# yangao07/LAMSA

Hardware: AMD Instinct MI355X
Metric: aligned Gbase/s, 10 kbp ONT-error reads (12%: sub/ins/del 4% each), -T ont2d vs GRCh37-sized stand-in; inputs resident in HBM when the timed region starts (upload excluded: see pcie_inclusive_*) (higher is better)
Workload: dtype int32

## Files before the change

### lamsa_amd/csrc/hp_align_api.hip

```cpp
#include <hip/hip_runtime.h>
#include <algorithm>
#include <atomic>
#include <map>
#include <mutex>
#include <stdlib.h>
#include <string.h>
#include <time.h>
#include "hp_phase.h"
#include "hp_handle.h"
#include "hp_hostprep.h"

using namespace hp;

#ifndef HP_WAVES_PER_SIMD
#define HP_WAVES_PER_SIMD 4
#endif
__global__ __launch_bounds__(64, HP_WAVES_PER_SIMD) void k_align_batch(AlignArgs a)
{
    __shared__ int32_t lds[HP_BOTH_LDS_WORDS];
    const int slot = blockIdx.x;
    for (;;) {
        int u = 0;
        if (wv::leader()) u = atomicAdd(a.counter, 1);
        u = wv::uni(u);
// ... 411 lines not shown
    S->valid = true;
    return LAMSA_HP_OK;
}

static int cap_waves(int n_waves, size_t slab_per_wave, int n_cu)
{
    static const size_t budget = []() { size_t f = 0, t = 0; if (hipMemGetInfo(&f, &t) != hipSuccess || t == 0) { t = (size_t)288 << 30; f = t; } return std::min(t / 4, f / 3); }();
    if (slab_per_wave * (size_t)n_waves <= budget) return n_waves;
    size_t fit = budget / (slab_per_wave ? slab_per_wave : 1);
    if (n_cu > 0 && fit >= (size_t)n_cu) fit -= fit % (size_t)n_cu;
    return fit < 1 ? 1 : (int)fit;
}

#ifdef HP_PROF
static void prof_report(Slot &T, const long long *d_prof, int n)
{
    if (!d_prof) return;
    {
        std::vector<long long> pr((size_t)n * 64);
        hipMemcpy(pr.data(), d_prof, sizeof(long long) * pr.size(), hipMemcpyDeviceToHost);
        if (const char *dump = getenv("LAMSA_HP_PROF_DUMP")) {
            if (FILE *fp = fopen(dump, "wb")) {
                for (int r = 0; r < n; ++r) { long long hl[2] = {T.h_H[r], T.h_len[r]}; fwrite(hl, 8, 2, fp); fwrite(&pr[(size_t)r * 64], 8, 64, fp); }
                fclose(fp);
            }
        }
        std::vector<int> idx((size_t)n); for (int i = 0; i < n; ++i) idx[i] = i;
        auto tot = [&](int r) { long long t = 0; for (int k = 0; k < 6; ++k) t += pr[(size_t)r * 64 + k]; return t; };
        std::sort(idx.begin(), idx.end(), [&](int x, int y) { return tot(x) > tot(y); });
        long long sum[64] = {0}; for (int r = 0; r < n; ++r) for (int k = 0; k < 64; ++k) sum[k] += pr[(size_t)r * 64 + k];
        fprintf(stderr, "[HP_PROF] cycles: setup chain1 fill1 chain2 fill2 publish | in chain1: init+minext mainscan track pop-loop bound+flines | o_l H\n");
        fprintf(stderr, "[HP_PROF] SUM  "); for (int k = 0; k < 11; ++k) fprintf(stderr, " %lld", sum[k] / 1000000); fprintf(stderr, " (Mcycles) targets %lld trips %lld init_Mcyc %lld\n", sum[11], sum[12], sum[13] / 1000000);
#ifdef HP_PROF_TRACK
        fprintf(stderr, "[HP_PROF] branch tracking (-DHP_PROF_TRACK: the line_build stamps below are off): marking pass %lld Mcyc; %lld seeds visited; %lld tracks, %lld Mcyc in them, %lld steps up; "
                        "%lld arrivals at a node with several sons, %lld Mcyc in cut_branch\n", sum[16] / 1000000, sum[19], sum[18], sum[17] / 1000000, sum[20], sum[21], sum[22] / 1000000);
#endif
        fprintf(stderr, "[HP_PROF] line_build: %lld lines (%lld without a gap), %lld anchors, %lld gaps | Mcyc: anchor walk %lld, gap list %lld, gaps in lanes %lld, gaps one by one %lld, assembly %lld\n",
                sum[21], sum[22], sum[12], sum[23], sum[16] / 1000000, sum[17] / 1000000, sum[18] / 1000000, sum[19] / 1000000, sum[20] / 1000000);
        fprintf(stderr, "[HP_PROF] gaps: %lld in lines with fewer than HP_GAP_MIN gaps (%lld lines with gaps); lane gaps: %lld hits scanned, %lld refused (range too long or too many active hits)\n", sum[54], sum[55], sum[11], sum[13]);
        { const char *nm[] = {"ksw_global", "ksw_extend", "backtrack", "ref_fetch", "head_fix", "frag_extend", "split_mapping", "tail_fix", "res_split", "res_aux", "mini_line_regs", "sort index"};
          for (int k = 0; k < 12; ++k) fprintf(stderr, "[HP_PROF] %-16s %8lld Mcyc %10lld calls\n", nm[k], sum[24 + 2 * k] / 1000000, sum[25 + 2 * k]);
#ifdef HP_PROF_FILL
          fprintf(stderr, "[HP_PROF] in frags_merge: boundary repair (merge_cigar_full) %lld Mcyc %lld calls; junctions through split_mapping %lld Mcyc %lld calls; fragments of several seeds %lld Mcyc %lld calls; 64-step gathers %lld Mcyc %lld\n", sum[16] / 1000000, sum[17], sum[18] / 1000000, sum[19], sum[20] / 1000000, sum[21], sum[22] / 1000000, sum[23]);
#endif
          fprintf(stderr, "[HP_PROF] direction-matrix bytes in HBM %lld (%lld jobs); hits passed through nodes_per_init %lld (%lld calls)\n", sum[52], sum[53], sum[54], sum[55]);
          fprintf(stderr, "[HP_PROF] chain_first start: seed loop %lld, node_set loop %lld, min_extend %lld Mcyc (%lld reads with a MIN pass)\n", sum[56] / 1000000, sum[57] / 1000000, sum[58] / 1000000, sum[59]);
          fprintf(stderr, "[HP_PROF] query <= 62: ksw_extend %lld Mcyc %lld calls, ksw_global %lld Mcyc %lld calls\n", sum[60] / 1000000, sum[61], sum[62] / 1000000, sum[63]);
          const char *bn[] = {"[bi_extend total]", "[bi_extend after left ext]", "17-32", "33-64", "65-128", "129-256", "257-512", ">512"};
          for (int k = 0; k < 2; ++k) fprintf(stderr, "[HP_PROF] ksw_extend qlen %-8s %8lld Mcyc %10lld calls\n", bn[k], sum[48 + 2 * k] / 1000000, sum[49 + 2 * k]); }
        {
            std::vector<long long> pd((size_t)n * 64);
            hipMemcpy(pd.data(), d_prof + ((size_t)n + 1) * 64, sizeof(long long) * pd.size(), hipMemcpyDeviceToHost);
            long long sd[64] = {0}; for (int r = 0; r < n; ++r) for (int k = 0; k < 64; ++k) sd[k] += pd[(size_t)r * 64 + k];
            const char *cn[] = {"one set, q <= 62", "packed, one set", "packed, two sets", "band 1 set slides", "band 2 sets slides", "band 4 sets slides", "int32 sets", "LDS / HBM rows",
                                "band 1 set fixed", "band 2 sets fixed", "band 4 sets fixed"};
            for (int c = 0; c < 11; ++c) fprintf(stderr, "[HP_PROF] wave jobs, ksw_extend %-18s %8lld Mcyc %10lld Mcells %9lld calls %10lld rows\n", cn[c], sd[4 * c] / 1000000, sd[4 * c + 1] / 1000000, sd[4 * c + 2], sd[4 * c + 3]);
            fprintf(stderr, "[HP_PROF] wave jobs, junctions of the class 'band 2 sets fixed': %lld jobs, wj_run %lld Mcyc of which staging %lld; ksw_bi_extend %lld Mcyc of which after the left extension %lld; "
                            "in ksw_extend_band<2>: setup and first fill %lld, rows %lld, backtrack %lld Mcyc\n",
                    sd[51], sd[50] / 1000000, sd[49] / 1000000, sd[47] / 1000000, sd[48] / 1000000, sd[44] / 1000000, sd[45] / 1000000, sd[46] / 1000000);
        }
        for (int q = 0; q < 8 && q < n; ++q) { int r = idx[q]; fprintf(stderr, "[HP_PROF] read %d L=%d:", r, T.h_len[r]); for (int k = 0; k < 11; ++k) fprintf(stderr, " %lld", pr[(size_t)r * 64 + k] / 1000000); fprintf(stderr, " | o_l %lld H %lld | targets %lld trips %lld init_Mcyc %lld\n", pr[(size_t)r * 64 + 14], pr[(size_t)r * 64 + 15], pr[(size_t)r * 64 + 11], pr[(size_t)r * 64 + 12], pr[(size_t)r * 64 + 13] / 1000000); }
    }
}
#endif

struct PhasedLayout { size_t bytes, o[15]; int unit_cap, lj_cap, wj_cap; int64_t fl_cap, line_cap, job_cap; };
static PhasedLayout phased_layout(int n, int64_t n_hits, int64_t n_bases, int64_t stream_cap)
// ... 193 lines not shown
    const int n = T.n_reads;
    for (float &v : h->kernel_ms) v = 0;
    S->r_st.assign((size_t)n + 1, 0); S->r_off.assign((size_t)n + 1, 0); S->r_len.assign((size_t)n + 1, 0); S->r_tb.assign((size_t)n + 1, 0); S->r_work.assign(4 * (size_t)n + 4, 0);
    if (S->stream.ensure(64)) { h->err = "hipHostMalloc(results)"; return LAMSA_HP_ENOMEM; }
    if (n == 0) {
        if (R) { R->stream = (const int32_t *)S->stream.p; R->stream_words = 0; R->read_off = S->r_off.data(); R->read_len = S->r_len.data(); R->read_status = S->r_st.data(); R->read_tbases = S->r_tb.data(); R->read_work = S->r_work.data(); }
        return LAMSA_HP_OK;
    }
    const double t_0 = now_s();
    HIPCHK(h, hipEventSynchronize(Ln.e1), LAMSA_HP_EKERNEL);
    const double t_1 = now_s();
    hipEventElapsedTime(&h->kernel_ms[0], Ln.e0, Ln.e1);
    if (Ln.phased) {
        hipEvent_t ev[6] = {Ln.e0, Ln.ep[0], Ln.ep[1], Ln.ep[2], Ln.ep[3], Ln.e1};
        for (int k = 0; k < 5; ++k) hipEventElapsedTime(&h->kernel_ms[2 + k], ev[k], ev[k + 1]);
        const unsigned long long *dg = Ln.out1.h_diag(n);
        for (int k = 0; k < 4; ++k) h->kernel_ms[7 + k] = dg[2 * k + 1] >= dg[2 * k] && dg[2 * k + 1] ? (float)((double)(dg[2 * k + 1] - dg[2 * k]) * 1e-5) : 0.f;
        h->kernel_ms[11] = (float)dg[8]; h->kernel_ms[12] = (float)dg[9];
        hipEventElapsedTime(&h->kernel_ms[13], Ln.ep[0], Ln.ep[4]);
        hipEventElapsedTime(&h->kernel_ms[14], Ln.ep[0], Ln.ep[5]);
        hipEventElapsedTime(&h->kernel_ms[15], Ln.ep[5], Ln.ep[6]);
        h->kernel_ms[16] = (float)dg[12]; h->kernel_ms[17] = (float)((double)dg[13] * 1e-6); h->kernel_ms[18] = (float)dg[14]; h->kernel_ms[19] = (float)((double)dg[15] * 4e-6); h->kernel_ms[20] = (float)((double)dg[16] * 1e-6);
#ifdef HP_PROF
        prof_report(T, (const long long *)Ln.prof.p, n);
#endif
    }
    memcpy(S->r_off.data(), Ln.out1.h_off(), 8 * (size_t)n); memcpy(S->r_len.data(), Ln.out1.h_len(n), 4 * (size_t)n);
    memcpy(S->r_st.data(), Ln.out1.h_st(n), 4 * (size_t)n); memcpy(S->r_tb.data(), Ln.out1.h_tb(n), 4 * (size_t)n); memcpy(S->r_work.data(), Ln.out1.h_work(n), 16 * (size_t)n);
    unsigned long long used1 = 0;
    for (int r = 0; r < n; ++r) if (S->r_off[r] >= 0 && (unsigned long long)(S->r_off[r] + S->r_len[r]) > used1) used1 = (unsigned long long)(S->r_off[r] + S->r_len[r]);
    if ((int64_t)used1 > Ln.out1.stream_cap) used1 = (unsigned long long)Ln.out1.stream_cap;
    std::vector<int32_t> again;
    for (int r = 0; r < n; ++r) if ((S->r_st[r] & LAMSA_HP_ST_OVERFLOW) || S->r_off[r] < 0) again.push_back(r);
    unsigned long long used2 = 0;
    if (!again.empty()) {
        int mL = 0, mH = 0; int64_t cap2 = 1024;
        for (int r : again) { mL = std::max(mL, T.h_len[r]); mH = std::max(mH, T.h_H[r]); cap2 += read_out_cap(T.h_len[r], 8, h->result_tags); }
        if (grow(h, S->out2.buf, 4 * (size_t)cap2 + 256) || S->out2.host.ensure(OutDev::hdr(n) + 256) || grow(h, S->retry_list, 4 * again.size())) { h->err = "hipMalloc(retry)"; return LAMSA_HP_ENOMEM; }
        S->out2.stream_cap = cap2;
        HIPCHK(h, hipMemcpyAsync(S->retry_list.p, again.data(), 4 * again.size(), hipMemcpyHostToDevice, Ln.cs), LAMSA_HP_EKERNEL);
        int rc = launch_align(h, S, T, Ln, S->out2, (const int32_t *)S->retry_list.p, (int)again.size(), 8, mL, mH, h->ev0, h->ev1, true);
        if (rc) return rc;
        hipEventElapsedTime(&h->kernel_ms[1], h->ev0, h->ev1);
        const int64_t *off2 = S->out2.h_off(); const int32_t *len2 = S->out2.h_len(n), *st2 = S->out2.h_st(n), *tb2 = S->out2.h_tb(n), *wk2 = S->out2.h_work(n);
        for (int r : again) if (off2[r] >= 0 && (unsigned long long)(off2[r] + len2[r]) > used2) used2 = (unsigned long long)(off2[r] + len2[r]);
        if ((int64_t)used2 > cap2) used2 = (unsigned long long)cap2;
        for (int r : again) { S->r_st[r] = st2[r]; S->r_len[r] = len2[r]; S->r_tb[r] = tb2[r]; for (int q = 0; q < 4; ++q) S->r_work[4 * r + q] = wk2[4 * r + q]; S->r_off[r] = off2[r] < 0 ? -1 : (int64_t)used1 + off2[r]; }
    }
    for (int r = 0; r < n; ++r) if (S->r_off[r] < 0) { S->r_off[r] = 0; S->r_len[r] = 0; S->r_st[r] |= LAMSA_HP_ST_OVERFLOW; }
    if (!R) return LAMSA_HP_OK;
    if (S->stream.ensure(4 * (size_t)(used1 + used2) + 64)) { h->err = "hipHostMalloc(results)"; return LAMSA_HP_ENOMEM; }
    int32_t *hs = (int32_t *)S->stream.p;
    if (used1) DL(hs, Ln.out1.stream(n), 4 * (size_t)used1);
    if (used2) DL(hs + used1, S->out2.stream(n), 4 * (size_t)used2);
    DLSYNC();
    if (g_trace) fprintf(stderr, "[lamsa_hp] collect: waited %.1f ms for the kernel (%.1f ms), results %.1f ms (%.2f GB)\n", 1e3 * (t_1 - t_0), h->kernel_ms[0], 1e3 * (now_s() - t_1), 4e-9 * (double)(used1 + used2));
    R->stream = hs; R->stream_words = (int64_t)(used1 + used2); R->read_off = S->r_off.data(); R->read_len = S->r_len.data(); R->read_status = S->r_st.data(); R->read_tbases = S->r_tb.data(); R->read_work = S->r_work.data();
    return LAMSA_HP_OK;
}
#undef DL
#undef DLSYNC

static int check_batch_args(lamsa_hp_handle *h, const lamsa_hp_batch *B)
{
    if (!h || !B || B->n_reads < 0) return LAMSA_HP_EINVAL;
    if (!h->d_pac) { h->err = "handle was created without a reference"; return LAMSA_HP_EINVAL; }
// ... 136 lines not shown
```

### lamsa_amd/csrc/hp_chain.h

```cpp
#pragma once
#include "hp_batch.h"
#include "hp_sort.h"

namespace hp {

enum { F_MATCH = 0, F_SPLIT_MATCH = 1, F_MISMATCH = 2, F_MATCH_THD = 2, F_LONG_MISMATCH = 3, F_INSERT = 4, F_DELETE = 5,
       F_CHR_DIF = 6, F_REVERSE = 7, F_UNCONNECT = 8, F_UNMATCH = 9, F_INIT = 20 };
enum { MIN_FLAG = 1, MULTI_FLAG = 2, UNLIMITED_FLAG = 3, WHOLE_FLAG = 4, TRACKED_FLAG = 5 };
enum { L_MERGB = 0, L_NMERG = 1, L_MERGH = 2, L_INTER = 4, L_DUMP = 8 };

HP_INL int score_table(int flag) { return flag <= 3 ? 1 : (flag <= 7 ? -3 : -6); }

#define HP_MAX_SLOTS 16383
#define HP_MAX_HITS_PER_SEED 16383

struct NodeS {
    int64_t pos;
    int32_t chr;
    int32_t slot_j;
    int16_t sid;
    int8_t strand, len_dif8;
    int8_t dp_flag;
    uint8_t son_flag;
    uint8_t match_flag;
// ... 509 lines not shown
{
    for (;;) {
        int l = 2 * i + 1, rr = 2 * (i + 1), m = i;
        if (l < ns.node_n && ns.node[l] < ns.node[i]) m = l;
        if (rr < ns.node_n && ns.node[rr] < ns.node[m]) m = rr;
        if (m == i) return;
        ns_swap(ns, i, m); i = m;
    }
}
HP_FN int ns_extract_minpos(NScore &ns)
{
    if (ns.node_n < 1) return -1;
    int m = ns.node[0];
    --ns.node_n;
    ns.node[0] = ns.node[ns.node_n]; ns.score[0] = ns.score[ns.node_n]; ns.NM[0] = ns.NM[ns.node_n];
    ns_minpos_sift(ns, 0);
    return m;
}
HP_FN int ns_add_bounded(NScore &ns, int node, int score, int NM)
{
    if (ns.node_n < ns.max_n) {
        ns.score[ns.node_n] = score; ns.NM[ns.node_n] = NM; ns.node[ns.node_n++] = node;
        if (ns.node_n == ns.max_n) for (int i = (ns.node_n - 1) / 2; i >= 0; --i) ns_min_sift(ns, i);
        return -1;
    }
    if (ns.score[0] < score || (ns.score[0] == score && ns.NM[0] > NM)) {
        int ret = ns.node[0];
        ns.score[0] = score; ns.NM[0] = NM; ns.node[0] = node;
        ns_min_sift(ns, 0);
        return ret;
    }
    return -2;
}
HP_FN void ns_add_end(ReadCtx &r, NScore &ns, int score, int NM, int node, const wv::Lane<int> *path = nullptr, int n_path = 0)
{
    if (score < ns.min_score_thd) return;
    if (ns.node_n >= ns.cap) { r.cx.status |= ST_OVERFLOW; return; }
    ns.score[ns.node_n] = score; ns.NM[ns.node_n] = NM; ns.node[ns.node_n++] = node;
    r.nd[node].dp_flag = TRACKED_FLAG;
    if (path) { HP_G NodeS *gd = (HP_G NodeS *)r.nd; WAVE_FOR(l) { if (l < n_path) gd[(*path)[l]].dp_flag = TRACKED_FLAG; } return; }
    for (int t = r.n_from[node]; t >= 0; t = r.n_from[t]) r.nd[t].dp_flag = TRACKED_FLAG;
}

HP_FN int best_son(ReadCtx &r, int f)
{
    int max_score = 0, max_NM = 0, max_dis = 0, flag_thd = F_INIT, max = -1;
    const int x = r.n_seed[f];
    for (int s = r.n_first[f], c = 0; c < r.n_son_n[f] && s >= 0; s = r.n_next[s], ++c) {
        const int mf = r.nd[s].match_flag, sx = r.n_seed[s];
        if (mf <= flag_thd && (r.n_max_score[s] > max_score || (r.n_max_score[s] == max_score && (sx - x < max_dis || r.n_max_NM[s] < max_NM)))) {
            max = s; max_score = r.n_max_score[s]; max_NM = r.n_max_NM[s]; max_dis = sx - x;
            if (mf <= F_MATCH_THD) flag_thd = F_MATCH_THD;
        }
    }
    return max;
}
HP_FN void detach(ReadCtx &r, int s, int max_node, NScore &ns)
{
    r.n_from[s] = -1;
    r.n_max_score[s] -= (r.nd[s].score - 1);
    r.n_max_NM[s] -= (r.nd[s].NM - r.h_nm[s]);
    r.n_node_n[max_node] -= (r.n_node_n[s] - 1);
    ns_add_end(r, ns, r.n_max_score[s], r.n_max_NM[s], max_node);
}
HP_INL void leaf_mark(ReadCtx &r, int f)
{
    if (r.leaf_on) { const int x = r.n_seed[f]; r.leaf_bits[x >> 5] |= (int)(1u << (x & 31)); }
}
HP_FN void cut_branch(ReadCtx &r, int f, NScore &ns)
{
    const int keep = best_son(r, f);
    if (keep < 0) { r.cx.status |= ST_REFEXIT; r.n_in_de[f] = 0; leaf_mark(r, f); return; }
    for (int s = r.n_first[f], c = 0, nn = r.n_son_n[f]; c < nn && s >= 0; ++c) {
        const int nxt = r.n_next[s];
        if (s != keep) detach(r, s, r.n_max_node[s], ns);
        s = nxt;
    }
    if (r.nd[f].score > r.n_max_score[keep]) {
        r.n_in_de[keep] = -1;
        detach(r, keep, r.n_max_node[keep], ns);
        r.n_son_n[f] = 0; r.n_first[f] = r.n_last[f] = -1;
        r.n_max_node[f] = f; r.n_max_score[f] = r.nd[f].score; r.n_max_NM[f] = r.nd[f].NM;
    } else {
        r.n_son_n[f] = 1; r.n_first[f] = r.n_last[f] = keep; r.n_next[keep] = -1;
        r.n_max_node[f] = r.n_max_node[keep]; r.n_max_score[f] = r.n_max_score[keep]; r.n_max_NM[f] = r.n_max_NM[keep];
    }
    r.n_in_de[f] = 0;
    leaf_mark(r, f);
}
HP_HOT void branch_track(ReadCtx &r, int n, NScore &ns)
{
    const HP_G int32_t *g_from = (const HP_G int32_t *)r.n_from, *g_son_n = (const HP_G int32_t *)r.n_son_n;
    const HP_G NodeS *g_nd = (const HP_G NodeS *)r.nd;
    HP_G int32_t *g_ms = (HP_G int32_t *)r.n_max_score, *g_mn = (HP_G int32_t *)r.n_max_NM, *g_mx = (HP_G int32_t *)r.n_max_node, *g_in_de = (HP_G int32_t *)r.n_in_de;
    int max_score, max_NM, max_node;
    g_in_de[n] = -1;
    const int n_sons = g_son_n[n], n_score = g_nd[n].score, n_NM = g_nd[n].NM;
    int fa = g_from[n];
    if (n_sons == 0) { max_node = n; max_score = n_score; max_NM = n_NM; }
    else { max_node = g_mx[n]; max_score = g_ms[n]; max_NM = g_mn[n]; }
    wv::Lane<int> path;
    WAVE_FOR(l) { path[l] = 0; }
    int n_path = 0; bool path_ok = n_sons == 0;
    int prev = n;
    while (fa >= 0) {
        const int fa_sons = g_son_n[fa], fa_score = g_nd[fa].score, fa_from = g_from[fa];
#ifdef HP_PROF_TRACK
        if (HP_PROF_CHAIN_ON && r.prof) r.prof[20] += 1;
#endif
        if (fa_sons == 1) {
            if (fa_score > max_score) {
                const int s = r.n_first[fa];
                g_ms[prev] = max_score; g_mn[prev] = max_NM; g_mx[prev] = max_node;
                wv::sync();
                r.n_in_de[s] = -1;
                detach(r, s, max_node, ns);
                r.n_son_n[fa] = 0; r.n_first[fa] = r.n_last[fa] = -1;
                max_score = r.nd[fa].score; max_NM = r.nd[fa].NM; max_node = fa;
                n_path = 0; path_ok = true;
            } else if (path_ok) {
                if (n_path < 64) { WAVE_FOR(l) { if (l == n_path) path[l] = fa; } ++n_path; } else path_ok = false;
            }
            prev = fa;
            fa = fa_from;
        } else {
            g_ms[prev] = max_score; g_mn[prev] = max_NM; g_mx[prev] = max_node;
            const int left_ = g_in_de[fa] - 1;
            g_in_de[fa] = left_;
#ifdef HP_PROF_TRACK
            if (HP_PROF_CHAIN_ON && r.prof) r.prof[21] += 1;
            const long long tcb_ = wv::clock();
#endif
            if (left_ == 0) { wv::sync(); cut_branch(r, fa, ns); }
#ifdef HP_PROF_TRACK
            if (HP_PROF_CHAIN_ON && r.prof) r.prof[22] += wv::clock() - tcb_;
#endif
            return;
        }
    }
    ns_add_end(r, ns, max_score, max_NM, max_node, path_ok ? &path : nullptr, n_path);
}

struct RunR { int lo, hi; };
HP_NOINL RunR reach_run(ReadCtx &r, int node, long long Rcap)
{
    const HP_G NodeS *ns = (const HP_G NodeS *)r.nd;
    const HP_G int32_t *g_srt = (const HP_G int32_t *)r.srt;
    const int H = r.H, rT = r.rnk[node];
    const NodeS N = node_load(ns + node);
    const int key = N.chr * 2 + (N.strand > 0 ? 1 : 0);
    int lo = rT, hi = rT;
    for (int dir = -1; dir <= 1; dir += 2) {
        int edge = rT;
        for (;;) {
            wv::Lane<int> bad;
            WAVE_FOR(l) {
                const int i = edge + dir * (1 + l), j = i - dir;
                int b = 1;
                if (i >= 0 && i < H) {
                    const NodeS A = node_load(ns + g_srt[i]), B = node_load(ns + g_srt[j]);
                    long long d = A.pos - B.pos; if (d < 0) d = -d;
                    b = !((A.chr * 2 + (A.strand > 0 ? 1 : 0)) == key && d <= Rcap);
                }
                bad[l] = b;
            }
            const unsigned long long m = wv::ballot(bad);
            if (m) { edge += dir * __builtin_ctzll(m); break; }
            edge += dir * 64;
        }
        if (dir < 0) lo = edge; else hi = edge;
    }
    RunR rr; rr.lo = lo; rr.hi = hi;
    return rr;
}

HP_INL void track_slot(ReadCtx &r, int h0, int h1, int dp_flag, bool skip_lone, NScore &ns)
{
    const HP_G NodeS *ns_ = (const HP_G NodeS *)r.nd;
    const HP_G int32_t *g_in_de = (const HP_G int32_t *)r.n_in_de, *g_from = (const HP_G int32_t *)r.n_from, *g_son_n = (const HP_G int32_t *)r.n_son_n;
    for (int b = h0; b < h1; b += 64) {
        wv::Lane<int> leaf;
        WAVE_FOR(l) {
            const int k = b + l;
            int v = 0;
            if (k < h1) {
                int q[4]; hp_load16((const HP_G char *)(ns_ + k) + 16, q); v = (int)(int8_t)(q[1] & 0xff) == dp_flag && g_in_de[k] == 0;
                if (v && skip_lone && g_from[k] < 0 && g_son_n[k] == 0) v = 0;
            }
            leaf[l] = v;
        }
        for (unsigned long long m = wv::ballot(leaf); m; m &= m - 1) {
#ifdef HP_PROF_TRACK
            const long long tb_ = wv::clock();
#endif
            branch_track(r, b + __builtin_ctzll(m), ns);
#ifdef HP_PROF_TRACK
            if (HP_PROF_CHAIN_ON && r.prof) { r.prof[17] += wv::clock() - tb_; r.prof[18] += 1; }
#endif
        }
    }
}
HP_NOINL void track_leaves(ReadCtx &r, int first_slot, int last_slot, int dp_flag, NScore &ns)
{
    const HP_G NodeS *ns_ = (const HP_G NodeS *)r.nd;
    const HP_G int32_t *g_in_de = (const HP_G int32_t *)r.n_in_de, *g_from = (const HP_G int32_t *)r.n_from, *g_son_n = (const HP_G int32_t *)r.n_son_n;
    const HP_G int32_t *g_seed = (const HP_G int32_t *)r.n_seed;
    const HP_G int64_t *g_hoff = (const HP_G int64_t *)r.hit_off;
    const int64_t hb = r.hb;
    const bool skip_lone = ns.min_score_thd > 1;
    if (last_slot < first_slot) return;
    const int nw = (last_slot >> 5) + 1, w_lo = first_slot >> 5;
    if (nw > r.cx.lds_words) {
        for (int i = last_slot; i >= first_slot; --i) track_slot(r, (int)(g_hoff[i] - hb), (int)(g_hoff[i + 1] - hb), dp_flag, skip_lone, ns);
        return;
    }
#ifdef HP_PROF_TRACK
    const long long tt0_ = wv::clock();
#endif
    HP_L int32_t *bits = r.cx.lds;
    for (int w0 = w_lo; w0 < nw; w0 += 64) { WAVE_FOR(l) { if (w0 + l < nw) bits[w0 + l] = 0; } }
    wv::sync();
    {
        const int k_lo = (int)(g_hoff[first_slot] - hb), k_hi = (int)(g_hoff[last_slot + 1] - hb);
        for (int b = k_lo; b < k_hi; b += 64) {
            WAVE_FOR(l) {
                const int k = b + l;
                if (k < k_hi) {
                    int q[4]; hp_load16((const HP_G char *)(ns_ + k) + 16, q);
                    int v = (int)(int8_t)(q[1] & 0xff) == dp_flag && g_in_de[k] == 0;
                    if (v && skip_lone && g_from[k] < 0 && g_son_n[k] == 0) v = 0;
                    if (v) { const int x = g_seed[k]; wv::lds_or(bits + (x >> 5), (int)(1u << (x & 31))); }
                }
            }
        }
    }
    wv::sync();
#ifdef HP_PROF_TRACK
    if (HP_PROF_CHAIN_ON && r.prof) r.prof[16] += wv::clock() - tt0_;
#endif
    r.leaf_bits = bits; r.leaf_on = true;
    for (int w = nw - 1; w >= w_lo; --w) {
        for (;;) {
            wv::sync();
            unsigned v = (unsigned)wv::uni(bits[w]);
            if (w == w_lo) v &= ~0u << (first_slot & 31);
            if (w == nw - 1 && (last_slot & 31) != 31) v &= (2u << (last_slot & 31)) - 1;
            if (!v) break;
            const int bit = 31 - __builtin_clz(v);
            wv::sync();
            bits[w] = (int)((unsigned)wv::uni(bits[w]) & ~(1u << bit));
            wv::sync();
            const int i = w * 32 + bit;
#ifdef HP_PROF_TRACK
            if (HP_PROF_CHAIN_ON && r.prof) r.prof[19] += 1;
#endif
            track_slot(r, (int)(g_hoff[i] - hb), (int)(g_hoff[i + 1] - hb), dp_flag, skip_lone, ns);
        }
    }
    r.leaf_on = false;
}

#define HP_MS_MAX_SETS 4
template <int NS> HP_INL int ms_pick(const wv::Lane<int> *f, int c) {
    const int l = c & 63, j = c >> 6;
    int v = wv::bcast(f[0], l);
#pragma unroll
    for (int q = 1; q < NS; ++q) { const int u = wv::bcast(f[q], l); v = j == q ? u : v; }
    return v;
}
struct MiniR { int n, d_score, d_NM; };
template <int NS>
HP_NOINL MiniR mini_line_sets(ReadCtx &r, int left, int right, int right_x, int32_t *line, int _head, int _tail,
                              int n_ids, const int32_t *list)
{
    left = wv::uni(left); right = wv::uni(right); right_x = wv::uni(right_x); _head = wv::uni(_head); _tail = wv::uni(_tail);
    const int head = _head ? left : -1;
    const int left_x = nx(r, left);
    const int dp_flag = MULTI_FLAG;
    const int start_slot = left_x + 1;
    const int k_lo = wv::uni(hoff(r, start_slot)), k_t0 = wv::uni(hoff(r, left_x + 2));
    const HP_G NodeS *ns = (const HP_G NodeS *)r.nd;
    HP_G NodeS *gd = (HP_G NodeS *)r.nd;
    const HP_G int16_t *g_hnm = (const HP_G int16_t *)r.h_nm;
    HP_G int32_t *g_from = (HP_G int32_t *)r.n_from, *g_node_n = (HP_G int32_t *)r.n_node_n;
    const EdgeK K = edge_consts(r.cx.P);
    const int POSMAX = (1 << 28) - 1;
    n_ids = wv::uni(n_ids);
    const HP_G int32_t *g_list = (const HP_G int32_t *)wv::uni64((long long)list);
    const bool by_list = list != nullptr;
    NodeS Fh; Fh.pos = 0; Fh.chr = 0; Fh.slot_j = 0; Fh.sid = 0; Fh.strand = 0; Fh.len_dif8 = 0; Fh.pad_ = 0; Fh.dp_flag = 0; Fh.son_flag = 0; Fh.match_flag = 0; Fh.score = 0; Fh.NM = 0;
    NodeS Rt = Fh;
    int head_nm = 0, right_nm = 0;
// ... 777 lines not shown
                WAVE_FOR(l) { const int c = c0 + l + 1; csn[l] = c <= C.n_cl ? g_cs[c] : H; }
                const bool geo32 = (long long)(r.seed_id[seed_out - 1] - r.seed_id[0] + 1) * P->seed_step <= 0x3fffffffll;
                if (geo32 && HP_CL_CAP_RT(1 << 20) >= HP_CLL_MCAP) {
                    const EdgeK K = edge_consts(P);
                    wv::sync();
                    WAVE_FOR(l) { const int n = csn[l] - csl[l]; if (l < cn && n >= 2 && n <= HP_CLL_MCAP) { HP_STAT_ADD(34, 1); HP_STAT_MAX(47, n); cluster_lane(r, K, C, r.cx.lds + l, csl[l], n, do_me); } }
                    wv::sync();
                }
                for (int q = 0; q < cn; ++q) {
                    const int lo = wv::bcast(csl, q), n = wv::bcast(csl, q + 1) - lo;
                    if (n < 2) continue;
                    if (geo32 && HP_CL_CAP_RT(1 << 20) >= HP_CLL_MCAP && n <= HP_CLL_MCAP) continue;
                    if (n <= HP_CL_CAP_RT(r.cx.lds_words / 5) && dp_cluster_lds(r, C, lo, n, do_me)) { HP_STAT_ADD(32, 1); HP_STAT_MAX(40, n); continue; }
                    HP_STAT_ADD(33, 1); HP_STAT_MAX(41, n);
                    if (do_me) min_extend_clusters(r, C, lo, lo + n);
                    for (int i0 = 0; i0 < n; i0 += 64) { WAVE_FOR(l) { if (i0 + l < n) g_big[g_srt[lo + i0 + l]] = 1; } }
                    any_big = true;
                }
            }
            wv::sync();
            if (any_big) dp_update_range(r, hoff(r, 1), H, 0, MIN_FLAG, false, false, C.big);
        }
        if (!have_cl) arena_release(r.cx.tmp, cmark);
        if (!build_sons(r, (HP_L uint64_t *)r.cx.lds, r.cx.lds_words / 2)) return false;
    }

    HP_CSTAMP(7);
#if defined(HP_CHAIN_STOP) && HP_CHAIN_STOP == 2
    return true;
#endif
    NScore &ns = loc->ns;
    if (!ns_alloc(r.cx, ns, H + 1, 0)) return false;
    ns.min_score_thd = 2;
    track_leaves(r, 0, seed_out - 1, MIN_FLAG, ns);

    HP_CSTAMP(8);
#if defined(HP_CHAIN_STOP) && HP_CHAIN_STOP == 3
    return true;
#endif
    const int o_l = ns.node_n;
    LSet &L = loc->L;
    Trig &T = loc->T;
    if (!lset_alloc(r.cx, L, 2 * H + o_l + 16, o_l)) return false;
    T.cap = 2 * H + 2 * o_l + 16; T.used = 0;
    T.n1 = (int32_t *)arena_alloc(r.cx, sizeof(int32_t) * (size_t)T.cap);
    T.n2 = (int32_t *)arena_alloc(r.cx, sizeof(int32_t) * (size_t)T.cap);
    T.off = (int32_t *)arena_alloc(r.cx, sizeof(int32_t) * (size_t)(o_l + 1));
    T.cnt = (int32_t *)arena_alloc(r.cx, sizeof(int32_t) * (size_t)(o_l + 1));
    int32_t *_line = (int32_t *)arena_alloc(r.cx, sizeof(int32_t) * (size_t)(H + 2));
    if (!T.n1 || !T.n2 || !T.off || !T.cnt || !_line) return false;
    const int l_i = lines_pop(r, ns, L, T, _line, have_cl ? &C : nullptr);
    if (l_i < 0) return false;
    L.n = l_i;
    HP_CSTAMP(9);
#if defined(HP_CHAIN_STOP) && HP_CHAIN_STOP == 4
    return true;
#endif
    LSet &S = loc->S;
    const bool staged = lset_stage(r, L, l_i, S);
    HP_STAT_ADD(staged ? 35 : 36, 1);
    HP_STAT_MAX(44, l_i);
    LSet &LL = staged ? S : L;
    const int line_n = set_bound(r, LL, 0, l_i, &T);
    const bool okf = build_flines(r, LL, line_n, F, fs);
    HP_CSTAMP(10);
    if (r.prof) { r.prof[14] = o_l; r.prof[15] = H; }
    return okf;
// ... 99 lines not shown
```

Baseline: 4.019.

## Track branches of the largest cluster in an LDS image instead of HBM

Before branch tracking, the largest seed cluster's node fields are packed into bit-packed words in LDS. Leaves in that cluster then run branch_track and cut_branch against the LDS image through a templated accessor, and the modified fields are written back to HBM afterwards. The aim is to replace the latency-bound pointer-chasing global loads and stores in the tracking walk with LDS accesses. In exchange it adds a build and write-back pass, validity checks that fall back to HBM, and bit-width limits on node fields.

Result: faster. 4.204 (median of 6 runs) (+4.6%).

```diff
diff --git a/lamsa_amd/csrc/hp_align_api.hip b/lamsa_amd/csrc/hp_align_api.hip
--- a/lamsa_amd/csrc/hp_align_api.hip
+++ b/lamsa_amd/csrc/hp_align_api.hip
@@ -467,7 +467,7 @@
         fprintf(stderr, "[HP_PROF] cycles: setup chain1 fill1 chain2 fill2 publish | in chain1: init+minext mainscan track pop-loop bound+flines | o_l H\n");
         fprintf(stderr, "[HP_PROF] SUM  "); for (int k = 0; k < 11; ++k) fprintf(stderr, " %lld", sum[k] / 1000000); fprintf(stderr, " (Mcycles) targets %lld trips %lld init_Mcyc %lld\n", sum[11], sum[12], sum[13] / 1000000);
 #ifdef HP_PROF_TRACK
-        fprintf(stderr, "[HP_PROF] branch tracking (-DHP_PROF_TRACK: the line_build stamps below are off): marking pass %lld Mcyc; %lld seeds visited; %lld tracks, %lld Mcyc in them, %lld steps up; "
+        fprintf(stderr, "[HP_PROF] branch tracking (-DHP_PROF_TRACK: the line_build stamps below are off): marking pass, image build and write-back %lld Mcyc; %lld seeds visited; %lld tracks, %lld Mcyc in them, %lld steps up; "
                         "%lld arrivals at a node with several sons, %lld Mcyc in cut_branch\n", sum[16] / 1000000, sum[19], sum[18], sum[17] / 1000000, sum[20], sum[21], sum[22] / 1000000);
 #endif
         fprintf(stderr, "[HP_PROF] line_build: %lld lines (%lld without a gap), %lld anchors, %lld gaps | Mcyc: anchor walk %lld, gap list %lld, gaps in lanes %lld, gaps one by one %lld, assembly %lld\n",
@@ -727,6 +727,9 @@
     if ((int64_t)used1 > Ln.out1.stream_cap) used1 = (unsigned long long)Ln.out1.stream_cap;
     std::vector<int32_t> again;
     for (int r = 0; r < n; ++r) if ((S->r_st[r] & LAMSA_HP_ST_OVERFLOW) || S->r_off[r] < 0) again.push_back(r);
+#ifdef HP_CHAIN_STOP
+    again.clear();
+#endif
     unsigned long long used2 = 0;
     if (!again.empty()) {
         int mL = 0, mH = 0; int64_t cap2 = 1024;
diff --git a/lamsa_amd/csrc/hp_chain.h b/lamsa_amd/csrc/hp_chain.h
--- a/lamsa_amd/csrc/hp_chain.h
+++ b/lamsa_amd/csrc/hp_chain.h
@@ -565,114 +565,9 @@
     }
     return -2;
 }
-HP_FN void ns_add_end(ReadCtx &r, NScore &ns, int score, int NM, int node, const wv::Lane<int> *path = nullptr, int n_path = 0)
-{
-    if (score < ns.min_score_thd) return;
-    if (ns.node_n >= ns.cap) { r.cx.status |= ST_OVERFLOW; return; }
-    ns.score[ns.node_n] = score; ns.NM[ns.node_n] = NM; ns.node[ns.node_n++] = node;
-    r.nd[node].dp_flag = TRACKED_FLAG;
-    if (path) { HP_G NodeS *gd = (HP_G NodeS *)r.nd; WAVE_FOR(l) { if (l < n_path) gd[(*path)[l]].dp_flag = TRACKED_FLAG; } return; }
-    for (int t = r.n_from[node]; t >= 0; t = r.n_from[t]) r.nd[t].dp_flag = TRACKED_FLAG;
-}
-
-HP_FN int best_son(ReadCtx &r, int f)
-{
-    int max_score = 0, max_NM = 0, max_dis = 0, flag_thd = F_INIT, max = -1;
-    const int x = r.n_seed[f];
-    for (int s = r.n_first[f], c = 0; c < r.n_son_n[f] && s >= 0; s = r.n_next[s], ++c) {
-        const int mf = r.nd[s].match_flag, sx = r.n_seed[s];
-        if (mf <= flag_thd && (r.n_max_score[s] > max_score || (r.n_max_score[s] == max_score && (sx - x < max_dis || r.n_max_NM[s] < max_NM)))) {
-            max = s; max_score = r.n_max_score[s]; max_NM = r.n_max_NM[s]; max_dis = sx - x;
-            if (mf <= F_MATCH_THD) flag_thd = F_MATCH_THD;
-        }
-    }
-    return max;
-}
-HP_FN void detach(ReadCtx &r, int s, int max_node, NScore &ns)
-{
-    r.n_from[s] = -1;
-    r.n_max_score[s] -= (r.nd[s].score - 1);
-    r.n_max_NM[s] -= (r.nd[s].NM - r.h_nm[s]);
-    r.n_node_n[max_node] -= (r.n_node_n[s] - 1);
-    ns_add_end(r, ns, r.n_max_score[s], r.n_max_NM[s], max_node);
-}
-HP_INL void leaf_mark(ReadCtx &r, int f)
-{
-    if (r.leaf_on) { const int x = r.n_seed[f]; r.leaf_bits[x >> 5] |= (int)(1u << (x & 31)); }
-}
-HP_FN void cut_branch(ReadCtx &r, int f, NScore &ns)
-{
-    const int keep = best_son(r, f);
-    if (keep < 0) { r.cx.status |= ST_REFEXIT; r.n_in_de[f] = 0; leaf_mark(r, f); return; }
-    for (int s = r.n_first[f], c = 0, nn = r.n_son_n[f]; c < nn && s >= 0; ++c) {
-        const int nxt = r.n_next[s];
-        if (s != keep) detach(r, s, r.n_max_node[s], ns);
-        s = nxt;
-    }
-    if (r.nd[f].score > r.n_max_score[keep]) {
-        r.n_in_de[keep] = -1;
-        detach(r, keep, r.n_max_node[keep], ns);
-        r.n_son_n[f] = 0; r.n_first[f] = r.n_last[f] = -1;
-        r.n_max_node[f] = f; r.n_max_score[f] = r.nd[f].score; r.n_max_NM[f] = r.nd[f].NM;
-    } else {
-        r.n_son_n[f] = 1; r.n_first[f] = r.n_last[f] = keep; r.n_next[keep] = -1;
-        r.n_max_node[f] = r.n_max_node[keep]; r.n_max_score[f] = r.n_max_score[keep]; r.n_max_NM[f] = r.n_max_NM[keep];
-    }
-    r.n_in_de[f] = 0;
-    leaf_mark(r, f);
-}
-HP_HOT void branch_track(ReadCtx &r, int n, NScore &ns)
-{
-    const HP_G int32_t *g_from = (const HP_G int32_t *)r.n_from, *g_son_n = (const HP_G int32_t *)r.n_son_n;
-    const HP_G NodeS *g_nd = (const HP_G NodeS *)r.nd;
-    HP_G int32_t *g_ms = (HP_G int32_t *)r.n_max_score, *g_mn = (HP_G int32_t *)r.n_max_NM, *g_mx = (HP_G int32_t *)r.n_max_node, *g_in_de = (HP_G int32_t *)r.n_in_de;
-    int max_score, max_NM, max_node;
-    g_in_de[n] = -1;
-    const int n_sons = g_son_n[n], n_score = g_nd[n].score, n_NM = g_nd[n].NM;
-    int fa = g_from[n];
-    if (n_sons == 0) { max_node = n; max_score = n_score; max_NM = n_NM; }
-    else { max_node = g_mx[n]; max_score = g_ms[n]; max_NM = g_mn[n]; }
-    wv::Lane<int> path;
-    WAVE_FOR(l) { path[l] = 0; }
-    int n_path = 0; bool path_ok = n_sons == 0;
-    int prev = n;
-    while (fa >= 0) {
-        const int fa_sons = g_son_n[fa], fa_score = g_nd[fa].score, fa_from = g_from[fa];
-#ifdef HP_PROF_TRACK
-        if (HP_PROF_CHAIN_ON && r.prof) r.prof[20] += 1;
-#endif
-        if (fa_sons == 1) {
-            if (fa_score > max_score) {
-                const int s = r.n_first[fa];
-                g_ms[prev] = max_score; g_mn[prev] = max_NM; g_mx[prev] = max_node;
-                wv::sync();
-                r.n_in_de[s] = -1;
-                detach(r, s, max_node, ns);
-                r.n_son_n[fa] = 0; r.n_first[fa] = r.n_last[fa] = -1;
-                max_score = r.nd[fa].score; max_NM = r.nd[fa].NM; max_node = fa;
-                n_path = 0; path_ok = true;
-            } else if (path_ok) {
-                if (n_path < 64) { WAVE_FOR(l) { if (l == n_path) path[l] = fa; } ++n_path; } else path_ok = false;
-            }
-            prev = fa;
-            fa = fa_from;
-        } else {
-            g_ms[prev] = max_score; g_mn[prev] = max_NM; g_mx[prev] = max_node;
-            const int left_ = g_in_de[fa] - 1;
-            g_in_de[fa] = left_;
-#ifdef HP_PROF_TRACK
-            if (HP_PROF_CHAIN_ON && r.prof) r.prof[21] += 1;
-            const long long tcb_ = wv::clock();
-#endif
-            if (left_ == 0) { wv::sync(); cut_branch(r, fa, ns); }
-#ifdef HP_PROF_TRACK
-            if (HP_PROF_CHAIN_ON && r.prof) r.prof[22] += wv::clock() - tcb_;
-#endif
-            return;
-        }
-    }
-    ns_add_end(r, ns, max_score, max_NM, max_node, path_ok ? &path : nullptr, n_path);
-}
+}
+#include "hp_track.h"
+namespace hp {
 
 struct RunR { int lo, hi; };
 HP_NOINL RunR reach_run(ReadCtx &r, int node, long long Rcap)
@@ -707,33 +602,42 @@
     return rr;
 }
 
-HP_INL void track_slot(ReadCtx &r, int h0, int h1, int dp_flag, bool skip_lone, NScore &ns)
-{
+template <bool RES>
+HP_INL void track_slot(ReadCtx &r, int h0, int h1, int dp_flag, bool skip_lone, NScore &ns, const TrImg &img)
+{
+    const HP_G int32_t *g_rnk = (const HP_G int32_t *)r.rnk;
     const HP_G NodeS *ns_ = (const HP_G NodeS *)r.nd;
     const HP_G int32_t *g_in_de = (const HP_G int32_t *)r.n_in_de, *g_from = (const HP_G int32_t *)r.n_from, *g_son_n = (const HP_G int32_t *)r.n_son_n;
     for (int b = h0; b < h1; b += 64) {
-        wv::Lane<int> leaf;
+        wv::Lane<int> leaf, place;
         WAVE_FOR(l) {
             const int k = b + l;
-            int v = 0;
+            int v = 0, pl = -1;
             if (k < h1) {
-                int q[4]; hp_load16((const HP_G char *)(ns_ + k) + 16, q); v = (int)(int8_t)(q[1] & 0xff) == dp_flag && g_in_de[k] == 0;
-                if (v && skip_lone && g_from[k] < 0 && g_son_n[k] == 0) v = 0;
-            }
-            leaf[l] = v;
+                if (RES && img.on) { const int p = g_rnk[k] - img.lo; if (p >= 0 && p < img.n) pl = p; }
+                if (pl >= 0) v = TrLds(r, img).leaf(pl, dp_flag, skip_lone);
+                else {
+                    int q[4]; hp_load16((const HP_G char *)(ns_ + k) + 16, q); v = (int)(int8_t)(q[1] & 0xff) == dp_flag && g_in_de[k] == 0;
+                    if (v && skip_lone && g_from[k] < 0 && g_son_n[k] == 0) v = 0;
+                }
+            }
+            leaf[l] = v; place[l] = pl;
         }
         for (unsigned long long m = wv::ballot(leaf); m; m &= m - 1) {
 #ifdef HP_PROF_TRACK
             const long long tb_ = wv::clock();
 #endif
-            branch_track(r, b + __builtin_ctzll(m), ns);
+            const int q_ = __builtin_ctzll(m), pl = RES && img.on ? wv::bcast(place, q_) : -1;
+            if (RES && pl >= 0) { HP_STAT_ADD(50, 1); branch_track(TrLds(r, img), r, pl, ns); }
+            else { if (RES && img.on) HP_STAT_ADD(51, 1); branch_track(TrHbm(r), r, b + q_, ns); }
 #ifdef HP_PROF_TRACK
             if (HP_PROF_CHAIN_ON && r.prof) { r.prof[17] += wv::clock() - tb_; r.prof[18] += 1; }
 #endif
         }
     }
 }
-HP_NOINL void track_leaves(ReadCtx &r, int first_slot, int last_slot, int dp_flag, NScore &ns)
+template <bool RES>
+HP_INL void track_leaves_on(ReadCtx &r, int first_slot, int last_slot, int dp_flag, NScore &ns, const TrImg &img)
 {
     const HP_G NodeS *ns_ = (const HP_G NodeS *)r.nd;
     const HP_G int32_t *g_in_de = (const HP_G int32_t *)r.n_in_de, *g_from = (const HP_G int32_t *)r.n_from, *g_son_n = (const HP_G int32_t *)r.n_son_n;
@@ -744,7 +648,7 @@
     if (last_slot < first_slot) return;
     const int nw = (last_slot >> 5) + 1, w_lo = first_slot >> 5;
     if (nw > r.cx.lds_words) {
-        for (int i = last_slot; i >= first_slot; --i) track_slot(r, (int)(g_hoff[i] - hb), (int)(g_hoff[i + 1] - hb), dp_flag, skip_lone, ns);
+        for (int i = last_slot; i >= first_slot; --i) track_slot<RES>(r, (int)(g_hoff[i] - hb), (int)(g_hoff[i + 1] - hb), dp_flag, skip_lone, ns, img);
         return;
     }
 #ifdef HP_PROF_TRACK
@@ -787,10 +691,18 @@
 #ifdef HP_PROF_TRACK
             if (HP_PROF_CHAIN_ON && r.prof) r.prof[19] += 1;
 #endif
-            track_slot(r, (int)(g_hoff[i] - hb), (int)(g_hoff[i + 1] - hb), dp_flag, skip_lone, ns);
+            track_slot<RES>(r, (int)(g_hoff[i] - hb), (int)(g_hoff[i + 1] - hb), dp_flag, skip_lone, ns, img);
         }
     }
     r.leaf_on = false;
+}
+HP_NOINL void track_leaves(ReadCtx &r, int first_slot, int last_slot, int dp_flag, NScore &ns)
+{
+    track_leaves_on<false>(r, first_slot, last_slot, dp_flag, ns, TrImg{0, 0, 0, 0});
+}
+HP_NOINL void track_leaves_img(ReadCtx &r, int first_slot, int last_slot, int dp_flag, NScore &ns, TrImg img)
+{
+    track_leaves_on<true>(r, first_slot, last_slot, dp_flag, ns, img);
 }
 
 #define HP_MS_MAX_SETS 4
@@ -1634,7 +1546,22 @@
     NScore &ns = loc->ns;
     if (!ns_alloc(r.cx, ns, H + 1, 0)) return false;
     ns.min_score_thd = 2;
-    track_leaves(r, 0, seed_out - 1, MIN_FLAG, ns);
+#ifdef HP_PROF_TRACK
+    const long long ti0_ = wv::clock();
+#endif
+    const TrImg img = have_cl && seed_out > 1 ? track_image_build(r, C.cs, C.n_cl, seed_out - 1) : TrImg{0, 0, 0, 0};
+#ifdef HP_PROF_TRACK
+    if (HP_PROF_CHAIN_ON && r.prof) r.prof[16] += wv::clock() - ti0_;
+#endif
+    if (img.on && all_min) HP_STAT_ADD(63, 1);
+    track_leaves_img(r, 0, seed_out - 1, MIN_FLAG, ns, img);
+#ifdef HP_PROF_TRACK
+    const long long ti1_ = wv::clock();
+#endif
+    if (img.on) track_image_store(r, img);
+#ifdef HP_PROF_TRACK
+    if (HP_PROF_CHAIN_ON && r.prof) r.prof[16] += wv::clock() - ti1_;
+#endif
 
     HP_CSTAMP(8);
 #if defined(HP_CHAIN_STOP) && HP_CHAIN_STOP == 3
diff --git a/lamsa_amd/csrc/hp_track.h b/lamsa_amd/csrc/hp_track.h
--- /dev/null
+++ b/lamsa_amd/csrc/hp_track.h
@@ -0,0 +1,295 @@
+#pragma once
+
+namespace hp {
+
+#ifndef HP_TRACK_MIN
+#define HP_TRACK_MIN 16
+#endif
+#define HP_TRACK_WORDS 6
+#define HP_TRACK_MAX_N 1020
+
+#ifdef __HIPCC__
+#define HP_MEM __device__ __forceinline__
+#else
+#define HP_MEM inline
+#endif
+
+struct TrImg { int on, lo, n, base; };
+
+struct TrHbm {
+    static constexpr bool IMG = false;
+    ReadCtx &r;
+    HP_G int32_t *g_from, *g_son_n, *g_in_de, *g_ms, *g_mn, *g_mx;
+    HP_G NodeS *gd;
+    HP_MEM TrHbm(ReadCtx &r_)
+        : r(r_), g_from((HP_G int32_t *)r_.n_from), g_son_n((HP_G int32_t *)r_.n_son_n), g_in_de((HP_G int32_t *)r_.n_in_de), g_ms((HP_G int32_t *)r_.n_max_score),
+          g_mn((HP_G int32_t *)r_.n_max_NM), g_mx((HP_G int32_t *)r_.n_max_node), gd((HP_G NodeS *)r_.nd) {}
+    HP_MEM int hit(int n) const { return n; }
+    HP_MEM int from(int n) const { return g_from[n]; }
+    HP_MEM int son_n(int n) const { return g_son_n[n]; }
+    HP_MEM int first(int n) const { return r.n_first[n]; }
+    HP_MEM int next(int n) const { return r.n_next[n]; }
+    HP_MEM int in_de(int n) const { return g_in_de[n]; }
+    HP_MEM int score(int n) const { return gd[n].score; }
+    HP_MEM int NM(int n) const { return gd[n].NM; }
+    HP_MEM int match_flag(int n) const { return r.nd[n].match_flag; }
+    HP_MEM int h_nm(int n) const { return r.h_nm[n]; }
+    HP_MEM int slot(int n) const { return r.n_seed[n]; }
+    HP_MEM int max_score(int n) const { return g_ms[n]; }
+    HP_MEM int max_NM(int n) const { return g_mn[n]; }
+    HP_MEM int max_node(int n) const { return g_mx[n]; }
+    HP_MEM int node_n(int n) const { return r.n_node_n[n]; }
+    HP_MEM void set_from(int n, int v) const { r.n_from[n] = v; }
+    HP_MEM void set_in_de(int n, int v) const { g_in_de[n] = v; }
+    HP_MEM void set_next(int n, int v) const { r.n_next[n] = v; }
+    HP_MEM void set_sons(int n, int cnt, int only) const { r.n_son_n[n] = cnt; r.n_first[n] = only; r.n_last[n] = only; }
+    HP_MEM void set_max_sn(int n, int s, int nm) const { g_ms[n] = s; g_mn[n] = nm; }
+    HP_MEM void set_max(int n, int s, int nm, int node) const { g_ms[n] = s; g_mn[n] = nm; g_mx[n] = node; }
+    HP_MEM void set_node_n(int n, int v) const { r.n_node_n[n] = v; }
+    HP_MEM void mark(int n) const { gd[n].dp_flag = TRACKED_FLAG; }
+    HP_MEM void marks_done() const {}
+};
+
+struct TrLds {
+    static constexpr bool IMG = true;
+    HP_L int32_t *w; int n, lo; const HP_G int32_t *g_srt;
+    HP_MEM TrLds(const ReadCtx &r, const TrImg &m) : w(r.cx.lds + m.base), n(m.n), lo(m.lo), g_srt((const HP_G int32_t *)r.srt) {}
+    HP_MEM int rd(int k, int i) const { return wv::uni(w[k * n + i]); }
+    HP_MEM void fld(int k, int i, int shift, int mask, int v) const { HP_L int32_t *p = w + k * n + i; *p = (*p & ~(mask << shift)) | ((v & mask) << shift); }
+    HP_MEM int hit(int i) const { return g_srt[lo + i]; }
+    HP_MEM int from(int i) const { return (rd(2, i) & 1023) - 1; }
+    HP_MEM int first(int i) const { return ((rd(2, i) >> 10) & 1023) - 1; }
+    HP_MEM int next(int i) const { return ((rd(2, i) >> 20) & 1023) - 1; }
+    HP_MEM int son_n(int i) const { return rd(3, i) & 1023; }
+    HP_MEM int in_de(int i) const { return ((rd(3, i) >> 10) & 2047) - 1; }
+    HP_MEM int max_node(int i) const { return (rd(3, i) >> 21) & 1023; }
+    HP_MEM int score(int i) const { return rd(0, i) >> 16; }
+    HP_MEM int NM(int i) const { return rd(0, i) & 0xffff; }
+    HP_MEM int max_score(int i) const { return rd(1, i) >> 16; }
+    HP_MEM int max_NM(int i) const { return rd(1, i) & 0xffff; }
+    HP_MEM int node_n(int i) const { return rd(4, i) & 2047; }
+    HP_MEM int h_nm(int i) const { return (rd(4, i) >> 11) & 0xffff; }
+    HP_MEM int slot(int i) const { return rd(5, i) & 16383; }
+    HP_MEM int match_flag(int i) const { return (rd(5, i) >> 14) & 31; }
+    HP_MEM void set_from(int i, int v) const { fld(2, i, 0, 1023, v + 1); }
+    HP_MEM void set_next(int i, int v) const { fld(2, i, 20, 1023, v + 1); }
+    HP_MEM void set_in_de(int i, int v) const { fld(3, i, 10, 2047, v + 1); }
+    HP_MEM void set_sons(int i, int cnt, int only) const { fld(3, i, 0, 1023, cnt); fld(2, i, 10, 1023, only + 1); }
+    HP_MEM void set_max_sn(int i, int s, int nm) const { w[n + i] = (int)(((unsigned)s << 16) | ((unsigned)nm & 0xffffu)); }
+    HP_MEM void set_max(int i, int s, int nm, int node) const { set_max_sn(i, s, nm); fld(3, i, 21, 1023, node); }
+    HP_MEM void set_node_n(int i, int v) const { fld(4, i, 0, 2047, v); }
+    HP_MEM void mark(int i) const { HP_L int32_t *p = w + 5 * n + i; *p = (*p & ~(15 << 19)) | (TRACKED_FLAG << 19); }
+    HP_MEM void marks_done() const { wv::sync(); }
+    HP_MEM int leaf(int i, int dp_flag, bool skip_lone) const {
+        const int lk = w[2 * n + i], ct = w[3 * n + i], id = w[5 * n + i];
+        int v = ((int)((unsigned)id << 9) >> 28) == dp_flag && ((ct >> 10) & 2047) == 1;
+        if (v && skip_lone && (lk & 1023) == 0 && (ct & 1023) == 0) v = 0;
+        return v;
+    }
+};
+
+template <class A>
+HP_HOT void ns_add_end(const A &a, ReadCtx &r, NScore &ns, int score, int NM, int node, const wv::Lane<int> *path = nullptr, int n_path = 0)
+{
+    if (score < ns.min_score_thd) return;
+    if (ns.node_n >= ns.cap) { r.cx.status |= ST_OVERFLOW; return; }
+    ns.score[ns.node_n] = score; ns.NM[ns.node_n] = NM; ns.node[ns.node_n++] = a.hit(node);
+    a.mark(node);
+    if (path) { WAVE_FOR(l) { if (l < n_path) a.mark((*path)[l]); } a.marks_done(); return; }
+    for (int t = a.from(node); t >= 0; t = a.from(t)) a.mark(t);
+}
+
+template <class A>
+HP_HOT int best_son(const A &a, int f)
+{
+    int max_score = 0, max_NM = 0, max_dis = 0, flag_thd = F_INIT, max = -1;
+    const int x = a.slot(f);
+    for (int s = a.first(f), c = 0, nn = a.son_n(f); c < nn && s >= 0; s = a.next(s), ++c) {
+        const int mf = a.match_flag(s), sx = a.slot(s), ms = a.max_score(s), mn = a.max_NM(s);
+        if (A::IMG && max >= 0) {
+            if (mf > flag_thd) HP_STAT_ADD(60, 1);
+            else if (ms == max_score && sx - x != max_dis) HP_STAT_ADD(58, 1);
+            else if (ms == max_score) HP_STAT_ADD(59, 1);
+        }
+        if (mf <= flag_thd && (ms > max_score || (ms == max_score && (sx - x < max_dis || mn < max_NM)))) {
+            max = s; max_score = ms; max_NM = mn; max_dis = sx - x;
+            if (mf <= F_MATCH_THD) flag_thd = F_MATCH_THD;
+        }
+    }
+    return max;
+}
+template <class A>
+HP_HOT void detach(const A &a, ReadCtx &r, int s, int max_node, NScore &ns)
+{
+    a.set_from(s, -1);
+    const int ms = a.max_score(s) - (a.score(s) - 1), mn = a.max_NM(s) - (a.NM(s) - a.h_nm(s));
+    a.set_max_sn(s, ms, mn);
+    a.set_node_n(max_node, a.node_n(max_node) - (a.node_n(s) - 1));
+    ns_add_end(a, r, ns, ms, mn, max_node);
+}
+template <class A>
+HP_HOT void leaf_mark(const A &a, ReadCtx &r, int f)
+{
+    if (r.leaf_on) { const int x = a.slot(f); r.leaf_bits[x >> 5] |= (int)(1u << (x & 31)); }
+}
+template <class A>
+HP_HOT void cut_branch(const A &a, ReadCtx &r, int f, NScore &ns)
+{
+    const int keep = best_son(a, f);
+    if (keep < 0) { r.cx.status |= ST_REFEXIT; a.set_in_de(f, 0); leaf_mark(a, r, f); return; }
+    const int nn = a.son_n(f);
+    if (A::IMG && nn >= 2) HP_STAT_ADD(53, 1);
+    if (A::IMG && nn >= 3) HP_STAT_ADD(62, 1);
+    for (int s = a.first(f), c = 0; c < nn && s >= 0; ++c) {
+        const int nxt = a.next(s);
+        if (s != keep) detach(a, r, s, a.max_node(s), ns);
+        s = nxt;
+    }
+    if (a.score(f) > a.max_score(keep)) {
+        if (A::IMG) HP_STAT_ADD(55, 1);
+        a.set_in_de(keep, -1);
+        detach(a, r, keep, a.max_node(keep), ns);
+        a.set_sons(f, 0, -1);
+        a.set_max(f, a.score(f), a.NM(f), f);
+    } else {
+        a.set_sons(f, 1, keep); a.set_next(keep, -1);
+        a.set_max(f, a.max_score(keep), a.max_NM(keep), a.max_node(keep));
+    }
+    a.set_in_de(f, 0);
+    leaf_mark(a, r, f);
+}
+template <class A>
+HP_HOT void branch_track(const A &a, ReadCtx &r, int n, NScore &ns)
+{
+    int max_score, max_NM, max_node;
+    a.set_in_de(n, -1);
+    const int n_sons = a.son_n(n), n_score = a.score(n), n_NM = a.NM(n);
+    int fa = a.from(n);
+    if (n_sons == 0) { max_node = n; max_score = n_score; max_NM = n_NM; }
+    else { max_node = a.max_node(n); max_score = a.max_score(n); max_NM = a.max_NM(n); }
+    wv::Lane<int> path;
+    WAVE_FOR(l) { path[l] = 0; }
+    int n_path = 0; bool path_ok = n_sons == 0;
+    int prev = n;
+    while (fa >= 0) {
+        const int fa_sons = a.son_n(fa), fa_score = a.score(fa), fa_from = a.from(fa);
+#ifdef HP_PROF_TRACK
+        if (HP_PROF_CHAIN_ON && r.prof) r.prof[20] += 1;
+#endif
+        if (A::IMG) HP_STAT_ADD(52, 1);
+        if (fa_sons == 1) {
+            if (fa_score > max_score) {
+                if (A::IMG) HP_STAT_ADD(54, 1);
+                const int s = a.first(fa);
+                a.set_max(prev, max_score, max_NM, max_node);
+                wv::sync();
+                a.set_in_de(s, -1);
+                detach(a, r, s, max_node, ns);
+                a.set_sons(fa, 0, -1);
+                max_score = a.score(fa); max_NM = a.NM(fa); max_node = fa;
+                n_path = 0; path_ok = true;
+            } else if (path_ok) {
+                if (n_path < 64) { WAVE_FOR(l) { if (l == n_path) path[l] = fa; } ++n_path; } else path_ok = false;
+            }
+            prev = fa;
+            fa = fa_from;
+        } else {
+            a.set_max(prev, max_score, max_NM, max_node);
+            const int left_ = a.in_de(fa) - 1;
+            a.set_in_de(fa, left_);
+#ifdef HP_PROF_TRACK
+            if (HP_PROF_CHAIN_ON && r.prof) r.prof[21] += 1;
+            const long long tcb_ = wv::clock();
+#endif
+            if (left_ == 0) { wv::sync(); cut_branch(a, r, fa, ns); }
+#ifdef HP_PROF_TRACK
+            if (HP_PROF_CHAIN_ON && r.prof) r.prof[22] += wv::clock() - tcb_;
+#endif
+            return;
+        }
+    }
+    if (A::IMG && !path_ok) HP_STAT_ADD(56, 1);
+    ns_add_end(a, r, ns, max_score, max_NM, max_node, path_ok ? &path : nullptr, n_path);
+}
+
+HP_NOINL TrImg track_image_build(ReadCtx &r, const int32_t *cs, int n_cl, int last_slot)
+{
+    TrImg m; m.on = 0; m.lo = 0; m.n = 0; m.base = 0;
+    const HP_G int32_t *g_cs = (const HP_G int32_t *)cs;
+    int n = 0, lo = 0;
+    for (int c0 = 0; c0 < n_cl; c0 += 64) {
+        wv::Lane<int> sz, e;
+        WAVE_FOR(l) { const int c = c0 + l; sz[l] = c < n_cl ? g_cs[c + 1] - g_cs[c] : 0; }
+        const int mx = wv::reduce_max(sz);
+        if (mx > n) { WAVE_FOR(l) e[l] = sz[l] == mx; n = mx; lo = g_cs[c0 + __builtin_ctzll(wv::ballot(e))]; }
+    }
+    const int nw = (last_slot >> 5) + 1;
+    if (last_slot < 0 || n < HP_TRACK_MIN || n > HP_TRACK_MAX_N || nw > r.cx.lds_words || HP_TRACK_WORDS * n > r.cx.lds_words - nw) return m;
+    const HP_G NodeS *ns_ = (const HP_G NodeS *)r.nd;
+    const HP_G int32_t *g_srt = (const HP_G int32_t *)r.srt, *g_rnk = (const HP_G int32_t *)r.rnk, *g_seed = (const HP_G int32_t *)r.n_seed;
+    const HP_G int32_t *g_from = (const HP_G int32_t *)r.n_from, *g_son_n = (const HP_G int32_t *)r.n_son_n, *g_first = (const HP_G int32_t *)r.n_first;
+    const HP_G int32_t *g_next = (const HP_G int32_t *)r.n_next, *g_in_de = (const HP_G int32_t *)r.n_in_de, *g_node_n = (const HP_G int32_t *)r.n_node_n;
+    const HP_G int16_t *g_hnm = (const HP_G int16_t *)r.h_nm;
+    HP_L int32_t *w = r.cx.lds + nw;
+    int nm_sum = 0, bad = 0;
+    wv::sync();
+    for (int i0 = 0; i0 < n; i0 += 64) {
+        wv::Lane<int> nml, badl;
+        WAVE_FOR(l) {
+            const int i = i0 + l;
+            int nmv = 0, bv = 0;
+            if (i < n) {
+                const int id = g_srt[lo + i];
+                int q[4]; hp_load16((const HP_G char *)(ns_ + id) + 16, q);
+                const int dpf = (int)(int8_t)(q[1] & 0xff), mf = (q[1] >> 16) & 0xff, score = q[2], NM = q[3];
+                const int fr = g_from[id], sn = g_son_n[id], fi = g_first[id], nx_ = g_next[id], ide = g_in_de[id], nn = g_node_n[id], slot = g_seed[id];
+                nmv = g_hnm[id];
+                const int pf = fr >= 0 ? g_rnk[fr] - lo : -1;
+                const int p1 = sn > 0 && fi >= 0 ? g_rnk[fi] - lo : -1;
+                const int pn = fr >= 0 && nx_ >= 0 ? g_rnk[nx_] - lo : -1;
+                bv = score < -30000 || score > 30000 || NM < 0 || NM > 65535 || nmv < 0 || sn < 0 || sn > n || (sn > 0 && fi < 0) || ide < 0 || ide > n ||
+                     nn < 1 || nn > n || slot < 0 || slot > 16383 || mf > 31 || dpf < -8 || dpf > 7 ||
+                     pf >= n || p1 >= n || pn >= n || (fr >= 0 && pf < 0) || (p1 < -1) || (pn < -1);
+                w[i] = (int)(((unsigned)score << 16) | ((unsigned)NM & 0xffffu));
+                w[n + i] = w[i];
+                w[2 * n + i] = ((pf + 1) & 1023) | (((p1 + 1) & 1023) << 10) | (((pn + 1) & 1023) << 20);
+                w[3 * n + i] = (sn & 1023) | (((ide + 1) & 2047) << 10) | (i << 21);
+                w[4 * n + i] = (nn & 2047) | ((nmv & 0xffff) << 11);
+                w[5 * n + i] = (slot & 16383) | ((mf & 31) << 14) | ((dpf & 15) << 19);
+            }
+            nml[l] = nmv; badl[l] = bv;
+        }
+        nm_sum += wv::reduce_sum(nml);
+        if (wv::ballot(badl) != 0) bad = 1;
+    }
+    wv::sync();
+    if (bad || nm_sum > 65535) { HP_STAT_ADD(61, 1); return m; }
+    HP_STAT_ADD(49, 1); HP_STAT_MAX(57, n);
+    m.on = 1; m.lo = lo; m.n = n; m.base = nw;
+    return m;
+}
+
+HP_NOINL void track_image_store(ReadCtx &r, TrImg m)
+{
+    const HP_G int32_t *g_srt = (const HP_G int32_t *)r.srt;
+    HP_G int32_t *g_from = (HP_G int32_t *)r.n_from, *g_node_n = (HP_G int32_t *)r.n_node_n;
+    HP_G NodeS *gd = (HP_G NodeS *)r.nd;
+    const HP_L int32_t *w = r.cx.lds + m.base;
+    const int n = m.n, lo = m.lo;
+    wv::sync();
+    for (int i0 = 0; i0 < n; i0 += 64) {
+        WAVE_FOR(l) {
+            const int i = i0 + l;
+            if (i < n) {
+                const int id = g_srt[lo + i];
+                const int fp = w[2 * n + i] & 1023;
+                g_from[id] = fp ? g_srt[lo + fp - 1] : -1;
+                g_node_n[id] = w[4 * n + i] & 2047;
+                gd[id].dp_flag = (int8_t)((int)((unsigned)w[5 * n + i] << 9) >> 28);
+            }
+        }
+    }
+    wv::sync();
+}
+
+}
```
